# befelix/safe_learning

Hardware: AMD Instinct MI355X
Metric: grid-cell Lyapunov checks/sec + ms/safe_set-update, 4D 128^4 grid, 1k-pt GP (higher is better)
Workload: dtype f64

## Files before the change

### include/sl_hip.h

```cpp
#ifndef SL_HIP_H
#define SL_HIP_H

#include <stdint.h>

#ifdef __cplusplus
extern "C" {
#endif

#define SL_API __attribute__((visibility("default")))

#define SL_OK               0
#define SL_ERR_INVALID     (-1)
#define SL_ERR_HIP         (-2)
#define SL_ERR_UNSUPPORTED (-3)
#define SL_ERR_NOMEM       (-4)

#define SL_MAX_STATE_DIM   6
#define SL_MAX_ACTION_DIM  2
#define SL_MAX_INPUT_DIM   8
#define SL_MAX_GP_HEADS    6
#define SL_MAX_NN_LAYERS   4
#define SL_MAX_SIMPLICES   32

typedef struct sl_ctx sl_ctx;
// ... 107 lines not shown

#define SL_POLYV_MAX_ENTRIES 256
SL_API int  sl_value_polynomial_set(sl_ctx* ctx, int d, int nterms, const double* h_coef,
                    const uint8_t* h_exponents, int normalize, const double* h_tx);

SL_API int  sl_gp_set_head(sl_ctx* ctx, int head, int n, int p, int dout, int col0,
                    const double* h_X, const double* h_Linv, const double* h_alpha,
                    double variance, const double* h_lengthscales);
#define SL_KERNEL_RBF 0
#define SL_KERNEL_MATERN32 1
#define SL_KERNEL_LINEAR 2
#define SL_KERNEL_MAX_FACTORS 8
typedef struct sl_gp_kernel_factor {
    int32_t kind, product;
    double  variance[SL_MAX_INPUT_DIM];
    double  inv_lengthscales[SL_MAX_INPUT_DIM];
} sl_gp_kernel_factor;
typedef struct sl_gp_kernel {
    int32_t nfactors, reserved;
    sl_gp_kernel_factor factor[SL_KERNEL_MAX_FACTORS];
} sl_gp_kernel;
SL_API int  sl_gp_set_head_kernel(sl_ctx* ctx, int head, int n, int p, int dout, int col0,
                    const double* h_X, const double* h_Linv, const double* h_alpha,
                    const sl_gp_kernel* h_kernel);
SL_API int  sl_gp_append_point(sl_ctx* ctx, int head, const double* h_x, const double* h_linv_row,
                        const double* h_alpha_new);
SL_API int  sl_gp_variance_floor(sl_ctx* ctx, int head, double* out, int n);
SL_API int  sl_gp_configure(sl_ctx* ctx, int nheads, double beta);
SL_API int  sl_gp4_early_configure(sl_ctx* ctx, int enable);
SL_API int  sl_gp4_workgroups_configure(sl_ctx* ctx, int workgroups);
SL_API int  sl_gp4_segment_configure(sl_ctx* ctx, int tiles);
SL_API int  sl_gp4_halves_configure(sl_ctx* ctx, int enable);
SL_API int  sl_gp4_predecide_configure(sl_ctx* ctx, int enable, int spacing);

SL_API int  sl_tri_set(sl_ctx* ctx, int slot, const sl_grid_desc* h_grid, int nsimplex,
                const int32_t* h_simplices, const double* h_hyperplanes,
                const double* h_discrete_points, int project, int ncols, const double* d_table);
SL_API int  sl_tri_set_table(sl_ctx* ctx, int slot, const double* d_table);

SL_API int  sl_network_set(sl_ctx* ctx, int nlayers, const int32_t* h_dims ,
                    const int32_t* h_activations, const double* h_kernels);

SL_API int  sl_policy_network_set(sl_ctx* ctx, int nlayers, const int32_t* h_dims,
                           const int32_t* h_activations, const double* h_kernels,
                           const double* h_biases, const int32_t* h_has_bias, double output_scale);

SL_API int  sl_values(sl_ctx* ctx, int64_t lo, int64_t hi, double* d_values);

SL_API int  sl_lyap_sweep(sl_ctx* ctx, int64_t lo, int64_t hi, const uint64_t* d_init_bits,
                   const double* d_values, uint64_t* d_neg_bits, sl_sweep_result* d_result,
                   double* d_dbg);


SL_API int  sl_values_implicit(sl_ctx* ctx, int* out);

SL_API int  sl_fold_results(sl_ctx* ctx, const sl_sweep_result* d_records, int count,
                     sl_sweep_result* d_out);

SL_API int  sl_lyap_finalize_dev(sl_ctx* ctx, int64_t lo, int64_t hi, const double* d_values,
                          const uint64_t* d_init_bits, const uint64_t* d_prev_bits,
                          const sl_sweep_result* d_folded, const sl_key* d_keep,
                          uint64_t* d_safe_bits, sl_sweep_result* d_result);

SL_API int  sl_refinement_carry(sl_ctx* ctx, int64_t lo, int64_t hi, const double* d_values,
                         const uint64_t* d_init_bits, const uint64_t* d_neg_bits,
                         const sl_sweep_result* d_folded, const sl_key* d_keep, int64_t* d_refinement);
// ... 166 lines not shown
```

### safe_learning_amd/_hip.py

```python

import ctypes as C
import os

import numpy as np

HERE = os.path.dirname(os.path.abspath(__file__))
LIB_PATH = os.environ.get("SL_LIB_PATH") or os.path.join(HERE, "libslhip.so")

MAX_STATE_DIM = 6
MAX_ACTION_DIM = 2
MAX_INPUT_DIM = 8
MAX_GP_HEADS = 6
MAX_NN_LAYERS = 4
MAX_SIMPLICES = 32

OK, ERR_INVALID, ERR_HIP, ERR_UNSUPPORTED, ERR_NOMEM = 0, -1, -2, -3, -4
POLICY_LINEAR, POLICY_CONST, POLICY_TABLE, POLICY_TRI, POLICY_NETWORK = 1, 2, 3, 4, 5
DYN_LINEAR, DYN_PENDULUM, DYN_CARTPOLE, DYN_GP, DYN_POLYNOMIAL = 1, 2, 3, 4, 5
POLY_MAX_TERMS, POLY_MAX_DEGREE = 64, 8
V_QUADRATIC, V_TRI, V_NETWORK, V_POLYNOMIAL = 1, 2, 3, 4
POLYV_MAX_ENTRIES = 256
LIP_CONST, LIP_ABS_LINEAR, LIP_NORM_LINEAR, LIP_ABS_GRAD, LIP_NORM_GRAD = 0, 1, 2, 3, 4
LF_CONST, LF_AFFINE_NORM1 = 0, 1
EVAL_VALUE, EVAL_POLICY, EVAL_DYNAMICS, EVAL_DECREASE, EVAL_LV, EVAL_GRADIENT = 1, 2, 3, 4, 5, 6
# ... 87 lines not shown
ADAPTIVE_ROW_WORDS = 6
SELECT_WORDS = 8
S_PREFIX, S_REMAINING, S_KEY_V, S_KEY_I, S_RANK, S_NONE = range(6)

_vp, _i64, _int, _dbl = C.c_void_p, C.c_int64, C.c_int, C.c_double
_int32_p = C.POINTER(C.c_int32)

SIGNATURES = {
    "sl_version": (_int, ()),
    "sl_ctx_create": (_int, (_int, _vp, C.POINTER(_vp))),
    "sl_ctx_destroy": (_int, (_vp,)),
    "sl_last_error": (C.c_char_p, (_vp,)),
    "sl_ctx_synchronize": (_int, (_vp,)),
    "sl_last_kernel": (C.c_char_p, (_vp,)),
    "sl_timing_configure": (_int, (_vp, _int)),
    "sl_timing_collect": (_int, (_vp, _int, c_double_p, _int, C.POINTER(_int))),
    "sl_model_set": (_int, (_vp, C.POINTER(ModelDesc))),
    "sl_policy_touch": (_int, (_vp,)),
    "sl_dynamics_polynomial_set": (_int, (_vp, _int, _int, _int, _int32_p, c_double_p, C.POINTER(C.c_uint8), _int,
                                          _dbl)),
    "sl_value_polynomial_set": (_int, (_vp, _int, _int, c_double_p, C.POINTER(C.c_uint8), _int, c_double_p)),
    "sl_gp_set_head": (_int, (_vp, _int, _int, _int, _int, _int, c_double_p, c_double_p, c_double_p, _dbl,
                              c_double_p)),
    "sl_gp_set_head_kernel": (_int, (_vp, _int, _int, _int, _int, _int, c_double_p, c_double_p, c_double_p,
                                     C.POINTER(GpKernel))),
    "sl_gp_append_point": (_int, (_vp, _int, c_double_p, c_double_p, c_double_p)),
    "sl_gp_variance_floor": (_int, (_vp, _int, c_double_p, _int)),
    "sl_gp_configure": (_int, (_vp, _int, _dbl)),
    "sl_gp4_early_configure": (_int, (_vp, _int)),
    "sl_gp4_workgroups_configure": (_int, (_vp, _int)),
    "sl_gp4_segment_configure": (_int, (_vp, _int)),
    "sl_gp4_halves_configure": (_int, (_vp, _int)),
    "sl_gp4_predecide_configure": (_int, (_vp, _int, _int)),
    "sl_tri_set": (_int, (_vp, _int, C.POINTER(GridDesc), _int, _int32_p, c_double_p, c_double_p, _int, _int,
                          _vp)),
    "sl_tri_set_table": (_int, (_vp, _int, _vp)),
    "sl_network_set": (_int, (_vp, _int, _int32_p, _int32_p, c_double_p)),
    "sl_policy_network_set": (_int, (_vp, _int, _int32_p, _int32_p, c_double_p, c_double_p, _int32_p, _dbl)),
    "sl_values": (_int, (_vp, _i64, _i64, _vp)),
    "sl_lyap_sweep": (_int, (_vp, _i64, _i64, _vp, _vp, _vp, _vp, _vp)),
    "sl_values_implicit": (_int, (_vp, C.POINTER(_int))),
    "sl_fold_results": (_int, (_vp, _vp, _int, _vp)),
    "sl_lyap_finalize_dev": (_int, (_vp, _i64, _i64, _vp, _vp, _vp, _vp, _vp, _vp, _vp)),
    "sl_refinement_carry": (_int, (_vp, _i64, _i64, _vp, _vp, _vp, _vp, _vp, _vp)),
    "sl_select_begin": (_int, (_vp, _vp, _i64, _i64, _vp, _i64)),
    "sl_select_hist": (_int, (_vp, _i64, _i64, _vp, _int, _int, _vp, _vp)),
    "sl_select_digit": (_int, (_vp, _int, _int, _vp, _vp)),
    "sl_sort_pairs": (_int, (_vp, _i64, _vp, _vp, _vp, _vp, _vp)),
    "sl_partition_by_digit": (_int, (_vp, _i64, _vp, _vp, _vp, _vp)),
    "sl_gather_rows": (_int, (_vp, _i64, _int, _vp, _vp, _vp)),
    "sl_adaptive_pack": (_int, (_vp, _i64, _i64, _vp, _vp, _int, _vp, _vp, _vp, _vp)),
    "sl_adaptive_dest": (_int, (_vp, _i64, _vp, _vp, _int, _vp)),
    "sl_adaptive_sort_keys": (_int, (_vp, _i64, _vp, _vp, _vp)),
    "sl_adaptive_analyse": (_int, (_vp, _i64, _i64, _i64, _vp, _vp, _dbl, _dbl, _i64, _vp, _vp)),
    "sl_adaptive_apply": (_int, (_vp, _i64, _i64, _i64, _vp, _vp, _vp, _dbl, _dbl, _i64, _vp)),
    "sl_adaptive_scatter": (_int, (_vp, _i64, _i64, _i64, _vp, _vp, _vp, _vp, _vp)),
    "sl_index_to_state": (_int, (_vp, _i64, _vp, _vp)),
    "sl_perturb_pairs": (_int, (_vp, _i64, _int, _int, _vp, _vp, _int, _vp, _vp, _vp)),
    "sl_rows_sort_key": (_int, (_vp, _i64, _int, _int, _vp, _vp, _vp)),
    "sl_rows_duplicate_flags": (_int, (_vp, _i64, _int, _vp, _vp, _vp)),
    "sl_sample_bounds": (_int, (_vp, _i64, _int, _int, _vp, _vp, _vp, _dbl, _vp, _vp)),
    "sl_state_membership": (_int, (_vp, _i64, _vp, _vp, _vp)),
    "sl_argmax_masked": (_int, (_vp, _i64, _vp, _vp, _vp)),
    "sl_argmax_rows_masked": (_int, (_vp, _i64, _int, _vp, _vp, _i64, _vp)),
    "sl_lyapunov_region": (_int, (_vp, _vp, _i64, _vp, _vp, C.POINTER(_int))),
    "sl_bits_to_bytes": (_int, (_vp, _i64, _vp, _vp)),
# ... 473 lines not shown

    def dense_param_grad(self, dims, activations, has_bias, output_scale, d_params, n, d, d_points, d_coeff, d_out):
        keep, (pd, pa, pb) = self._dense_description(dims, activations, has_bias)
        self.lib.sl_dense_param_grad(self.handle, len(keep[1]), pd, pa, pb, float(output_scale), _ptr(d_params),
                                     int(n), int(d), _ptr(d_points), _ptr(d_coeff), _ptr(d_out))

    def nn_train_scratch(self):
        nbytes, intact = _i64(0), _int(0)
        self.lib.sl_debug_nn_train_scratch(self.handle, C.byref(nbytes), C.byref(intact))
        return int(nbytes.value), bool(intact.value)

    def synchronize(self):
        self.lib.sl_ctx_synchronize(self.handle)

    TIMING_LYAP_SWEEP, TIMING_FINALIZE, TIMING_BELLMAN = 0, 1, 2

    def timing_configure(self, slots):
        self.lib.sl_timing_configure(self.handle, int(slots))
        self._timing_slots = int(slots)

    def timing_collect(self, channel):
        slots = getattr(self, "_timing_slots", 0)
        if not slots:
            return []
        out = (C.c_double * slots)()
        count = C.c_int(0)
        self.lib.sl_timing_collect(self.handle, int(channel), out, slots, C.byref(count))
        return [float(out[i]) for i in range(count.value)]

    def last_kernel(self):
        name = self.lib.sl_last_kernel(self.handle)
        return name.decode() if name else ""

    @staticmethod
    def comm_unique_id():
        lib = load_library()
        buf = C.create_string_buffer(128)
        rc = lib.sl_comm_unique_id(buf)
        if rc != 0:
            raise HipEngineError("sl_comm_unique_id failed: %s" % lib.sl_last_error(None).decode())
        return buf.raw

    def comm_init(self, unique_id, rank, world):
        self.lib.sl_comm_init(self.handle, unique_id, rank, world)

    def comm_destroy(self):
        self.lib.sl_comm_destroy(self.handle)

    def allreduce_result(self, d_result):
        self.lib.sl_allreduce_result(self.handle, _ptr(d_result))

    def allgather(self, d_send, d_recv, nbytes):
        self.lib.sl_allgather(self.handle, _ptr(d_send), _ptr(d_recv), nbytes)

    def allreduce_sum_u64(self, d_values, count):
        self.lib.sl_allreduce_sum_u64(self.handle, _ptr(d_values), count)

    def allreduce_max_f64(self, d_values, count):
        self.lib.sl_allreduce_max_f64(self.handle, _ptr(d_values), count)

    def debug_mfma(self, a, b):
        a, pa = _as_c(a)
        b, pb = _as_c(b)
        out = np.zeros((16, 16))
        self.lib.sl_debug_mfma(self.handle, pa, pb, out.ctypes.data_as(c_double_p))
        return out
# ... 24 lines not shown
```

### safe_learning_amd/csrc/sl_gp4_mean.hip

```cpp
#include "sl_common.h"
#include "sl_gp4_gen.h"
#include "sl_gp4_mean.h"
#include "sl_gp4_predecide.h"
#include "sl_gp4_queue.h"

#ifndef SL_NO_GP4

namespace gp4m {

using gp4::RUNC;
using gp4::RUNS;
using gp4::uniform;

constexpr int W = 4;
constexpr int WG_PER_CU = 4;
constexpr int KXS2 = 128 + 4;
constexpr int KXBUF = 8 * KXS2;
constexpr int SLICE = KXBUF + 16 * SL_P + RUNS * RUNC;
static_assert(16 * SL_D <= KXBUF, "the block's means reuse the chunk buffer");
static_assert(W * SLICE * sizeof(double) <= 40 * 1024, "four workgroups of k_gp_mean_blocks per CU");

}

#ifdef SL_DIAG
static __device__ unsigned long long sl_gp4_mean_decided;
#endif

template <int DT, int MT>
__global__ __launch_bounds__(256, 4) void k_gp_mean_blocks(
    const SlDevModel M, const SlGpDev gp, SlAux aux, int64_t lo, int64_t hi, int64_t tile0, int64_t tile1,
    const uint64_t* __restrict__ init_bits, const double* __restrict__ values,
    uint64_t* __restrict__ neg_bits, sl_key* __restrict__ partials, int fold,
    const double* __restrict__ points, int skip_arg, unsigned long long* __restrict__ ticket,
    unsigned* __restrict__ list_count, long long* __restrict__ list_cell, double* __restrict__ list_mean,
    unsigned list_cap, const unsigned char* __restrict__ pre_tiles) {
#ifdef SL_DIAG
    const int skip = skip_arg;
#else
    constexpr int skip = 0;
    (void)skip_arg;
#endif
    using namespace gp4m;
    __shared__ __attribute__((aligned(16))) double smem[W * SLICE];
    const SlDims nd = sl_dims<DT, MT>(M);
    const int d = nd.d, p = nd.p;
    const int tid = threadIdx.x, lane = tid & 63;
    const int wave = __builtin_amdgcn_readfirstlane(tid >> 6);
    const int lcol = lane & 15, lk = lane >> 4, blk = (lane >> 2) & 3, low = lane & 3;
    double* kx_l = smem + wave * SLICE;
    double* cell_mean = kx_l;
    double* cin = kx_l + KXBUF;
    double* runc = cin + 16 * SL_P;
    const int own = 2 * (16 * lk + ((lcol + 4 * (lk >> 1)) & 15));
// ... 179 lines not shown
                const int64_t b16 = (blk0 - lo) >> 4;
                unsigned init = 0u;
                if (init_bits) init = reinterpret_cast<const unsigned short*>(init_bits)[b16];
                if (lane == 0) reinterpret_cast<unsigned short*>(neg_bits)[b16] = (unsigned short)word;
                const bool okc = neg_hi || ((init >> lcol) & 1u);
                if (valid && !okc) sl_key_min(best_v, best_i, sl_vbits(v_x), idx);
#ifdef SL_DIAG
                if (lane == 0) atomicAdd(&sl_gp4_mean_decided, 1ull);
#endif
            } else {
                unsigned at = 0u;
                if (lane == 0) at = atomicAdd(list_count, 1u);
                at = (unsigned)__builtin_amdgcn_readfirstlane((int)at);
                if (at < list_cap) {
                    if (lane == 0) list_cell[at] = blk0;
                    double* rec = list_mean + (size_t)at * 16 * d;
                    for (int i = lane; i < 16 * d; i += 64) rec[i] = cell_mean[(i / d) * SL_D + i % d];
                }
            }
            __builtin_amdgcn_fence(__ATOMIC_RELEASE, "wavefront");
            __builtin_amdgcn_wave_barrier();
        }
    }
    sl_wave_reduce_key<true>(best_v, best_i);
    if (lane == 0) {
        sl_key* out = partials + blockIdx.x * W + wave;
        if (fold) sl_key_min(best_v, best_i, out->vbits, out->index);
        out->vbits = best_v;
        out->index = best_i;
    }
}

template <int DT, int MT>
static int launch_mean(sl_ctx* ctx, const SlDevModel& model, const SlSweepArgs& a, const Gp4MeanLaunch& m) {
    SlAux aux{ctx->d_tri, ctx->d_net};
    const int skip = sl_diag_flags("SL_GP4_SKIP");
    if (!m.fold) {
        ctx->gp4_pre_tiles = nullptr;
        ctx->gp4_pre_count = nullptr;
        if (sl_gp4_predecide_ok(ctx, model, a)) {
            const Gp4PreLaunch pl{m.workgroups, m.partials, m.ticket + 5};
            const int rc = sl_gp4_predecide_launch_dim<DT>(ctx, model, a, pl, &ctx->gp4_pre_tiles);
            if (rc) return rc;
            ctx->gp4_pre_count = m.ticket + 5;
        }
    }
    const int fold = m.fold || ctx->gp4_pre_tiles != nullptr;
    hipLaunchKernelGGL((k_gp_mean_blocks<DT, MT>), dim3((unsigned)m.workgroups), dim3(gp4m::W * 64), 0, ctx->stream,
                       model, ctx->h_gp, aux, a.lo, a.hi, (int64_t)m.tile0, (int64_t)m.tile1, a.init_bits, a.values,
                       a.neg_bits, m.partials, fold, a.points, skip, m.ticket, m.list_count, m.list_cell,
                       m.list_mean, m.list_cap, ctx->gp4_pre_tiles);
    SL_HIP_CHECK(ctx, hipGetLastError());
    return SL_OK;
}

#if !defined(SL_GP4_DIM) || SL_GP4_DIM == 4
int sl_gp4_mean_workgroups(const sl_ctx* ctx, long long tiles) {
    long long wg = (long long)ctx->num_cu * gp4m::WG_PER_CU;
    const long long need = (tiles + gp4m::W - 1) / gp4m::W;
    if (wg > need) wg = need;
    if (wg > SL_MAX_GRID / 2) wg = SL_MAX_GRID / 2;
    return (int)(wg < 1 ? 1 : wg);
}

unsigned long long sl_gp4_mean_decided_fetch(sl_ctx* ctx) {
    unsigned long long c = 0ull;
#ifdef SL_DIAG
    if (hipMemcpyFromSymbol(&c, HIP_SYMBOL(sl_gp4_mean_decided), sizeof(c)) != hipSuccess) return 0ull;
    const unsigned long long zero = 0ull;
    (void)hipMemcpyToSymbol(HIP_SYMBOL(sl_gp4_mean_decided), &zero, sizeof(zero));
#endif
    (void)ctx;
    return c;
}
#endif

#define SL_GP4_MEAN_ENTRY(D_)                                                                                \
    template <>                                                                                              \
    int sl_gp4_mean_launch_dim<D_>(sl_ctx* ctx, const SlDevModel& model, const SlSweepArgs& a,               \
                                   const Gp4MeanLaunch& m) {                                                 \
// ... 16 lines not shown
```

### safe_learning_amd/csrc/sl_gp4_predecide.h

```cpp
#pragma once
#include "sl_model.h"

namespace gp4p {

constexpr double SLACK = 0x1p-40;
constexpr long long MAX_LATTICE = 1ll << 24;
constexpr long long MAX_TABLE_BYTES = 64ll << 20;

struct PreConst {
    double norm[SL_D], eps[SL_D];
    double sdev;
    int32_t spacing, count[SL_D];
};

SL_HD int row_doubles(int d, int p) { return p + d + d * p; }
SL_HD int lattice_count(int num, int S) { return (num - 1 + S - 1) / S + 1; }
SL_HD int lattice_grid_index(int a, int num, int S) { return a * S < num - 1 ? a * S : num - 1; }
SL_HD int lattice_nearest(int i, int num, int S) {
    const int a = i / S, ia = a * S;
    const int ib = ia + S < num - 1 ? ia + S : num - 1;
    return (i - ia) > (ib - i) ? a + 1 : a;
}

constexpr double HALF_SQRT3 = 0.8660254037844388;
// ... 31 lines not shown
                   0x1p-48 * absm;
            A[j] = fabs(mu[j]) + B[j];
        }
    }
    double vc = 0.0, lin = 0.0, quad = 0.0, mag = 0.0;
#pragma unroll
    for (int j = 0; j < SL_D; ++j) {
        if (j < d) {
            double row = 0.0, grad = 0.0, qb = 0.0, qa = 0.0;
#pragma unroll
            for (int i = 0; i < SL_D; ++i) {
                if (i < d) {
                    row = row + mu[i] * v.matrix[i][j];
                    grad = grad + mu[i] * (v.matrix[i][j] + v.matrix[j][i]);
                    qb = qb + fabs(v.matrix[i][j]) * B[i];
                    qa = qa + fabs(v.matrix[i][j]) * A[i];
                }
            }
            vc = vc + row * mu[j];
            lin = lin + fabs(grad) * B[j];
            quad = quad + qb * B[j];
            mag = mag + qa * A[j];
        }
    }
    mag = mag + fabs(v_x) + fabs(thr);
    const double lower = ((vc - lin) - quad) - v_x;
    return mag < INFINITY && lower >= thr + SLACK * mag;
}

}

#if defined(__HIPCC__)
#include "sl_common.h"

struct Gp4PreLaunch {
    int workgroups;
    sl_key* partials;
    unsigned long long* decided;
};

bool sl_gp4_predecide_ok(const sl_ctx* ctx, const SlDevModel& model, const SlSweepArgs& a);

template <int D>
int sl_gp4_predecide_launch_dim(sl_ctx* ctx, const SlDevModel& model, const SlSweepArgs& a, const Gp4PreLaunch& m,
                                const unsigned char** tiles);
#define SL_GP4_PRE_DECL(D_)                                                                                  \
    template <> int sl_gp4_predecide_launch_dim<D_>(sl_ctx*, const SlDevModel&, const SlSweepArgs&,          \
                                                    const Gp4PreLaunch&, const unsigned char**);
SL_GP4_PRE_DECL(1) SL_GP4_PRE_DECL(2) SL_GP4_PRE_DECL(3) SL_GP4_PRE_DECL(4)
#undef SL_GP4_PRE_DECL
#endif
```

### safe_learning_amd/csrc/sl_gp4_predecide.hip

```cpp
#include "sl_common.h"
#include "sl_gp4_predecide.h"

template <int DT, int MT>
__global__ __launch_bounds__(256) void k_gp_mean_lattice(const SlDevModel M, const SlGpDev gp, SlAux aux,
                                                         const gp4p::PreConst pc, long long npoints,
                                                         double* __restrict__ table) {
    const SlDims nd = sl_dims<DT, MT>(M);
    const int d = nd.d, p = nd.p;
    const SlGpHeadDev& hd = gp.head[0];
    const long long at = (long long)blockIdx.x * blockDim.x + threadIdx.x;
    if (at >= npoints) return;
    long long r = at;
    int64_t cell = 0, stride = 1;
#pragma unroll
    for (int k = SL_D - 1; k >= 0; --k) {
        if (k < d) {
            const int a = (int)(r % pc.count[k]);
            r /= pc.count[k];
            cell += stride * gp4p::lattice_grid_index(a, M.m.grid.num_points[k], pc.spacing);
            stride *= M.m.grid.num_points[k];
        }
    }
    double xg[SL_P], u[SL_M], g[SL_D], J[SL_D][SL_P];
    sl_cell_state(M, d, cell, nullptr, xg);
// ... 81 lines not shown
        double z_c[SL_P], g_c[SL_D], J[SL_D * SL_P];
#pragma unroll
        for (int q = 0; q < SL_P; ++q) z_c[q] = (q < p) ? row[q] : 0.0;
#pragma unroll
        for (int j = 0; j < SL_D; ++j) g_c[j] = (j < d) ? row[p + j] : 0.0;
#pragma unroll
        for (int i = 0; i < SL_D * SL_P; ++i) J[i] = (i < d * p) ? row[p + d + i] : 0.0;
        const bool sure = valid && gp4p::sure_fail(M.m.value, d, p, pc, z, z_c, g_c, J, prior, v_x, thr);
        const uint64_t ok = __ballot(sure || !valid);
        unsigned dec = 0u;
#pragma unroll
        for (int jb = 0; jb < 4; ++jb)
            if (((ok >> (16 * jb)) & 0xffffull) == 0xffffull) dec |= 1u << jb;
        const bool mine = (dec >> (lane >> 4)) & 1u;
        if (mine && (lane & 15) == 0) reinterpret_cast<unsigned short*>(neg_bits)[4 * t + (lane >> 4)] = (unsigned short)0;
        bool init = false;
        if (init_bits && valid) init = (init_bits[t] >> lane) & 1ull;
        if (valid && mine && !init) sl_key_min(best_v, best_i, sl_vbits(values ? values[idx - lo] : v_x), idx);
        if (lane == 0) tiles[t] = (unsigned char)dec;
        const int64_t left = hi - (lo + 64 * t);
        const unsigned live = left >= 64 ? 15u : (1u << (int)((left + 15) >> 4)) - 1u;
        count += (unsigned)__builtin_popcount(dec & live);
    }
    sl_wave_reduce_key<true>(best_v, best_i);
    if (lane == 0) {
        sl_key* out = partials + blockIdx.x * 4 + wave;
        out->vbits = best_v;
        out->index = best_i;
        if (count) atomicAdd(decided, (unsigned long long)count);
    }
}

#if !defined(SL_GP4_DIM) || SL_GP4_DIM == 4
constexpr int64_t PRE_MIN_TILES = 1 << 15;

bool sl_gp4_predecide_ok(const sl_ctx* ctx, const SlDevModel& model, const SlSweepArgs& a) {
    if (ctx->gp4_segment_tiles <= 0 && (a.hi - a.lo + 63) / 64 < PRE_MIN_TILES) return false;
    if (!ctx->gp4_predecide || ctx->gp4_pre_spacing < 1 || a.points || a.dbg || ctx->h_gp.nheads != 1) return false;
    const SlGpHeadHost& hh = ctx->gp_heads[0];
    if (!hh.set || !hh.mb_ok || hh.d_kernel || hh.col0 != 0 || hh.dout != model.m.grid.d) return false;
    if (model.m.value.kind != SL_V_QUADRATIC || model.m.value.negate) return false;
    if (model.m.policy.kind != SL_POLICY_LINEAR && model.m.policy.kind != SL_POLICY_CONST) return false;
    long long npoints = 1;
    for (int k = 0; k < model.m.grid.d; ++k) {
        if (model.m.grid.num_points[k] < 1) return false;
        npoints *= gp4p::lattice_count((int)model.m.grid.num_points[k], ctx->gp4_pre_spacing);
        if (npoints > gp4p::MAX_LATTICE) return false;
    }
    const int d = model.m.grid.d;
    if (npoints * gp4p::row_doubles(d, model.in_dim) * (long long)sizeof(double) > gp4p::MAX_TABLE_BYTES) return false;
    return true;
}

extern "C" int sl_gp4_predecide_configure(sl_ctx* ctx, int enable, int spacing) {
    if (!ctx) return sl_fail(nullptr, SL_ERR_INVALID, "sl_gp4_predecide_configure: NULL context");
    if (spacing < 0 || spacing > 4096)
        return sl_fail(ctx, SL_ERR_INVALID, "sl_gp4_predecide_configure: spacing %d outside [0,4096]", spacing);
    ctx->gp4_predecide = enable != 0;
    if (spacing > 0) ctx->gp4_pre_spacing = spacing;
    return SL_OK;
}
#endif

template <int DT, int MT>
static int launch_predecide(sl_ctx* ctx, const SlDevModel& model, const SlSweepArgs& a, const Gp4PreLaunch& m,
                            const unsigned char** tiles_out) {
    const SlGpHeadHost& hh = ctx->gp_heads[0];
    gp4p::PreConst pc = {};
    long long npoints = 1;
    for (int k = 0; k < DT; ++k) {
        pc.norm[k] = hh.mb_norm[k];
        pc.eps[k] = hh.mb_eps[k];
        pc.count[k] = gp4p::lattice_count((int)model.m.grid.num_points[k], ctx->gp4_pre_spacing);
        npoints *= pc.count[k];
    }
    pc.spacing = ctx->gp4_pre_spacing;
    pc.sdev = sqrt(ctx->h_gp.head[0].variance) * (1.0 + 0x1p-50);
    const int64_t ntiles = (a.hi - a.lo + 63) / 64;
    const size_t table_bytes = ((size_t)npoints * gp4p::row_doubles(DT, DT + MT) * sizeof(double) + 255) & ~(size_t)255;
    SL_HIP_CHECK(ctx, sl_grow(ctx, &ctx->d_gp4_pre, &ctx->gp4_pre_bytes, table_bytes + (size_t)ntiles + 4));
    double* table = reinterpret_cast<double*>(ctx->d_gp4_pre);
    unsigned char* tiles = reinterpret_cast<unsigned char*>(ctx->d_gp4_pre) + table_bytes;
    SlAux aux{ctx->d_tri, ctx->d_net};
    hipLaunchKernelGGL((k_gp_mean_lattice<DT, MT>), dim3((unsigned)((npoints + 255) / 256)), dim3(256), 0, ctx->stream,
                       model, ctx->h_gp, aux, pc, npoints, table);
    SL_HIP_CHECK(ctx, hipGetLastError());
    hipLaunchKernelGGL((k_gp_predecide<DT, MT>), dim3((unsigned)m.workgroups), dim3(256), 0, ctx->stream, model,
                       ctx->h_gp, aux, pc, a.lo, a.hi, a.init_bits, a.values, a.neg_bits, m.partials, table, tiles,
                       m.decided);
    SL_HIP_CHECK(ctx, hipGetLastError());
    *tiles_out = tiles;
    return SL_OK;
}

#define SL_GP4_PRE_ENTRY(D_)                                                                                 \
    template <>                                                                                              \
    int sl_gp4_predecide_launch_dim<D_>(sl_ctx* ctx, const SlDevModel& model, const SlSweepArgs& a,          \
                                        const Gp4PreLaunch& m, const unsigned char** tiles) {                \
        return launch_predecide<D_, 1>(ctx, model, a, m, tiles);                                             \
    }
#if !defined(SL_GP4_DIM) || SL_GP4_DIM == 1
SL_GP4_PRE_ENTRY(1)
#endif
#if !defined(SL_GP4_DIM) || SL_GP4_DIM == 2
SL_GP4_PRE_ENTRY(2)
#endif
#if !defined(SL_GP4_DIM) || SL_GP4_DIM == 3
SL_GP4_PRE_ENTRY(3)
#endif
#if !defined(SL_GP4_DIM) || SL_GP4_DIM == 4
SL_GP4_PRE_ENTRY(4)
#endif
```

Measured before the change: 313.4 million.

## Compact predecided tiles into an open-block list and sweep only open blocks

After the predecide pass, two new kernels count and scatter the indices of still-open 16-cell blocks into a compact list using a chunked prefix sum. A new k_gp_mean_open kernel walks this list through an atomic ticket, so the expensive GP mean evaluation runs only on undecided blocks rather than scanning every tile and skipping decided ones. This adds two small kernel launches, extra device memory and an indirection, and it changes how tiles are assigned to workgroups. A host API to read back the open list is also added for inspection.

Result: faster. 329.2 million (median of 6 runs) (+5.0%).

```diff
diff --git a/include/sl_hip.h b/include/sl_hip.h
--- a/include/sl_hip.h
+++ b/include/sl_hip.h
@@ -163,6 +163,7 @@
 SL_API int  sl_gp4_segment_configure(sl_ctx* ctx, int tiles);
 SL_API int  sl_gp4_halves_configure(sl_ctx* ctx, int enable);
 SL_API int  sl_gp4_predecide_configure(sl_ctx* ctx, int enable, int spacing);
+SL_API int  sl_gp4_open_list(sl_ctx* ctx, uint32_t* out, int64_t cap, unsigned long long* count, int* used);
 
 SL_API int  sl_tri_set(sl_ctx* ctx, int slot, const sl_grid_desc* h_grid, int nsimplex,
                 const int32_t* h_simplices, const double* h_hyperplanes,
diff --git a/safe_learning_amd/_hip.py b/safe_learning_amd/_hip.py
--- a/safe_learning_amd/_hip.py
+++ b/safe_learning_amd/_hip.py
@@ -143,6 +143,7 @@
     "sl_gp4_segment_configure": (_int, (_vp, _int)),
     "sl_gp4_halves_configure": (_int, (_vp, _int)),
     "sl_gp4_predecide_configure": (_int, (_vp, _int, _int)),
+    "sl_gp4_open_list": (_int, (_vp, C.POINTER(C.c_uint32), _i64, C.POINTER(C.c_ulonglong), C.POINTER(_int))),
     "sl_tri_set": (_int, (_vp, _int, C.POINTER(GridDesc), _int, _int32_p, c_double_p, c_double_p, _int, _int,
                           _vp)),
     "sl_tri_set_table": (_int, (_vp, _int, _vp)),
@@ -682,6 +683,18 @@
         name = self.lib.sl_last_kernel(self.handle)
         return name.decode() if name else ""
 
+    def gp4_open_list(self, entries=True):
+        import numpy as np
+        count, used = C.c_ulonglong(0), C.c_int(0)
+        self.lib.sl_gp4_open_list(self.handle, None, 0, C.byref(count), C.byref(used))
+        if not entries:
+            return int(count.value), bool(used.value)
+        out = np.zeros(int(count.value), dtype=np.uint32)
+        if len(out):
+            self.lib.sl_gp4_open_list(self.handle, out.ctypes.data_as(C.POINTER(C.c_uint32)), len(out),
+                                      C.byref(count), C.byref(used))
+        return out, bool(used.value)
+
     @staticmethod
     def comm_unique_id():
         lib = load_library()
diff --git a/safe_learning_amd/csrc/sl_gp4_mean.hip b/safe_learning_amd/csrc/sl_gp4_mean.hip
--- a/safe_learning_amd/csrc/sl_gp4_mean.hip
+++ b/safe_learning_amd/csrc/sl_gp4_mean.hip
@@ -19,6 +19,9 @@
 constexpr int SLICE = KXBUF + 16 * SL_P + RUNS * RUNC;
 static_assert(16 * SL_D <= KXBUF, "the block's means reuse the chunk buffer");
 static_assert(W * SLICE * sizeof(double) <= 40 * 1024, "four workgroups of k_gp_mean_blocks per CU");
+constexpr int KEYS = 2 * 16;
+constexpr int SLICE_OPEN = SLICE + KEYS;
+static_assert(W * SLICE_OPEN * sizeof(double) <= 40 * 1024, "four workgroups of k_gp_mean_open per CU");
 
 }
 
@@ -264,6 +267,251 @@
 }
 
 template <int DT, int MT>
+__global__ __launch_bounds__(256, 4) void k_gp_mean_open(
+    const SlDevModel M, const SlGpDev gp, SlAux aux, int64_t lo, int64_t hi, unsigned p0, unsigned p1,
+    const unsigned* __restrict__ open_list, const unsigned long long* __restrict__ open_len,
+    const uint64_t* __restrict__ init_bits, const double* __restrict__ values,
+    uint64_t* __restrict__ neg_bits, sl_key* __restrict__ partials,
+    const double* __restrict__ points, int skip_arg, unsigned* __restrict__ ticket,
+    unsigned* __restrict__ list_count, long long* __restrict__ list_cell, double* __restrict__ list_mean,
+    unsigned list_cap) {
+#ifdef SL_DIAG
+    const int skip = skip_arg;
+#else
+    constexpr int skip = 0;
+    (void)skip_arg;
+#endif
+    using namespace gp4m;
+    __shared__ __attribute__((aligned(16))) double smem[W * SLICE_OPEN];
+    const SlDims nd = sl_dims<DT, MT>(M);
+    const int d = nd.d, p = nd.p;
+    const int tid = threadIdx.x, lane0 = tid & 63;
+    const int wave = __builtin_amdgcn_readfirstlane(tid >> 6);
+    double* kx_l = smem + wave * SLICE_OPEN;
+    double* cell_mean = kx_l;
+    double* cin = kx_l + KXBUF;
+    double* runc = cin + 16 * SL_P;
+    uint64_t* keys = reinterpret_cast<uint64_t*>(runc + RUNS * RUNC);
+    if (lane0 < 16) {
+        keys[2 * lane0] = ~0ull;
+        keys[2 * lane0 + 1] = (uint64_t)INT64_MAX;
+    }
+
+    const SlGpHeadDev& hd = gp.head[0];
+    const int n_pad = hd.n_pad, dout = hd.dout;
+    const double variance = hd.variance;
+    __amdgpu_buffer_rsrc_t rs_xs = __builtin_amdgcn_make_buffer_rsrc((void*)hd.xs, 0, 0x7fffffff, 0x27000);
+    __amdgpu_buffer_rsrc_t rs_alpha = __builtin_amdgcn_make_buffer_rsrc((void*)hd.alpha, 0, 0x7fffffff, 0x27000);
+    constexpr int RP = 256;
+    const int npanels = (hd.n + RP - 1) / RP;
+    const int nchunks_head = npanels * (RP / 64);
+
+    {
+        const unsigned long long len = open_len[0];
+        if (len < (unsigned long long)p1) p1 = (unsigned)len;
+    }
+    if (p0 >= p1) return;
+    auto request = [&]() -> unsigned {
+        unsigned t = 0u;
+        if (lane0 == 0) t = atomicInc(ticket, 0xffffffffu);
+        return t;
+    };
+    unsigned drawn = request();
+    for (;;) {
+        asm volatile("" : "+v"(drawn));
+        const unsigned pos = p0 + 4u * (unsigned)__builtin_amdgcn_readfirstlane((int)drawn);
+        if (pos >= p1) break;
+        drawn = request();
+        const sl_u4 entry = *reinterpret_cast<const sl_u4*>(open_list + pos);
+        const int nb = p1 - pos < 4u ? (int)(p1 - pos) : 4;
+        for (int jb = 0; jb < nb; ++jb) {
+            const unsigned b16 = jb == 0 ? entry.x : jb == 1 ? entry.y : jb == 2 ? entry.z : entry.w;
+            const int64_t blk0 = lo + 16 * (int64_t)b16;
+            int lane = lane0;
+            asm volatile("" : "+v"(lane));
+            const int lcol = lane & 15, lk = lane >> 4, blk = (lane >> 2) & 3, low = lane & 3;
+            const int own = 2 * (16 * lk + ((lcol + 4 * (lk >> 1)) & 15));
+            const int wbase = (lane >> 3) * KXS2 + 32 * (lane & 3) + ((lane >> 2) & 1);
+            const int wswz = 4 * ((lane & 3) >> 1);
+            if (lk == 0) {
+                double xg[SL_P], u[SL_M];
+                int64_t gidx = blk0 + lcol;
+                gidx = gidx < hi ? gidx : hi - 1;
+                sl_cell_state(M, d, gidx, points, xg);
+                sl_policy_any<false>(M, nd, aux.tri, gidx, xg, u);
+                sl_append_action(nd, u, xg);
+#pragma unroll
+                for (int q = 0; q < SL_P; ++q) cin[lcol * SL_P + q] = (q < p) ? xg[q] * hd.inv_ls[q] : 0.0;
+            }
+            __builtin_amdgcn_fence(__ATOMIC_RELEASE, "wavefront");
+            __builtin_amdgcn_wave_barrier();
+            unsigned runs = 1u;
+            bool wide = false;
+            {
+                bool bend = false;
+                if (lcol >= 1) {
+                    double st2 = 0.0;
+#pragma unroll
+                    for (int q = 0; q < SL_P; ++q) {
+                        if (q < p) {
+                            const double st = cin[lcol * SL_P + q] - cin[(lcol - 1) * SL_P + q];
+                            st2 = fma(st, st, st2);
+                        }
+                    }
+                    wide = !(st2 <= 1.0);
+                }
+                if (lcol >= 2) {
+#pragma unroll
+                    for (int q = 0; q < SL_P; ++q) {
+                        if (q < p) {
+                            const double c0 = cin[lcol * SL_P + q];
+                            const double c1 = cin[(lcol - 1) * SL_P + q];
+                            const double c2 = cin[(lcol - 2) * SL_P + q];
+                            bend = bend || fabs((c0 - c1) - (c1 - c2)) > 2e-14 * fmax(1.0, fabs(c0));
+                        }
+                    }
+                }
+                unsigned bends = (unsigned)(__ballot(bend) & 0xffffull);
+                while (bends) {
+                    const int c = __builtin_ctz(bends);
+                    runs |= 1u << c;
+                    bends &= ~(3u << c);
+                }
+            }
+            runs = (unsigned)__builtin_amdgcn_readfirstlane((int)runs);
+            const bool direct = __builtin_popcount(runs) > 4 || (__ballot(wide) & 0xffffull) != 0ull;
+            if (!direct || runs == 1u) {
+                if (lane < RUNS) {
+                    unsigned m = runs;
+                    for (int r = 0; r < lane; ++r) m &= m - 1;
+                    if (m) {
+                        const int c0 = __builtin_ctz(m);
+                        m &= m - 1;
+                        const int c1 = m ? __builtin_ctz(m) : 16;
+                        const double* at = cin + c0 * SL_P;
+                        const bool single = c1 - c0 < 2;
+                        double a2r = 0.0;
+                        double* rc = runc + lane * RUNC;
+#pragma unroll
+                        for (int q = 0; q < SL_P; ++q) {
+                            const double step = (q < p && !single) ? at[SL_P + q] - at[q] : 0.0;
+                            rc[q] = step;
+                            a2r = fma(step, step, a2r);
+                        }
+                        rc[SL_P] = a2r;
+                        rc[SL_P + 1] = sl_exp_nonpos(-a2r);
+                    }
+                }
+                __builtin_amdgcn_fence(__ATOMIC_RELEASE, "wavefront");
+                __builtin_amdgcn_wave_barrier();
+            }
+            double macc[4] = {0.0, 0.0, 0.0, 0.0};
+
+            auto generate = [&](int ch) {
+                double* kxw = kx_l + wbase;
+                double xv[SL_P];
+#pragma unroll
+                for (int q = 0; q < SL_P; ++q)
+                    if (q < p)
+                        xv[q] = __builtin_bit_cast(double, __builtin_amdgcn_raw_buffer_load_b64(
+                            rs_xs, lane * 8, (q * n_pad + 64 * ch) * 8, 0));
+                if (runs == 1u) {
+                    double e, rho;
+                    gp4::run_seed(xv, cin, runc, variance, p, e, rho);
+                    gp4::store_run16(kxw, wswz, rho, e, runc[SL_P + 1]);
+                } else if (!direct) {
+                    unsigned m = runs;
+                    for (int r = 0; m; ++r) {
+                        const int c0 = __builtin_ctz(m);
+                        m &= m - 1;
+                        const int c1 = m ? __builtin_ctz(m) : 16;
+                        const double* rc = runc + r * RUNC;
+                        double e, rho;
+                        gp4::run_seed(xv, cin + c0 * SL_P, rc, variance, p, e, rho);
+                        const double qr = rc[SL_P + 1];
+                        for (int c = c0; c < c1; ++c) {
+                            kxw[2 * ((c + wswz) & 15)] = e;
+                            e *= rho;
+                            rho *= qr;
+                        }
+                    }
+                } else {
+                    gp4::direct_run(kxw, wswz, xv, cin, 0, variance, p);
+                }
+            };
+            for (int ch = 0; ch < nchunks_head; ++ch) {
+                const bool with_mean = !(skip & 2);
+                gp4::MeanIn mi;
+                if (with_mean) gp4::load_alpha(mi, rs_alpha, lk, low, dout, ch);
+                if (!(skip & 1)) generate(ch);
+                if (with_mean) {
+                    __builtin_amdgcn_fence(__ATOMIC_RELEASE, "wavefront");
+                    __builtin_amdgcn_wave_barrier();
+                    sl_d2 kx[8];
+                    gp4::load_own_kx<KXS2>(kx, kx_l + own);
+                    gp4::mean_mfma(kx, mi, macc);
+                }
+            }
+            __builtin_amdgcn_fence(__ATOMIC_RELEASE, "wavefront");
+            __builtin_amdgcn_wave_barrier();
+            if (lk < dout) cell_mean[(4 * blk + low) * SL_D + hd.col0 + lk] = gp4::mean_sum(macc);
+            __builtin_amdgcn_fence(__ATOMIC_RELEASE, "wavefront");
+            __builtin_amdgcn_wave_barrier();
+
+            const int64_t idx = blk0 + lcol;
+            const bool valid = lk == 0 && idx < hi;
+            gp4::CellBounds b{false, false, 0.0};
+            if (valid)
+                b = gp4::cell_bounds<false>(M, nd, aux, gp.beta, idx, lo, points, values, cell_mean + lcol * SL_D, variance,
+                                            0.0, 0.0);
+            const bool neg_hi = b.neg_hi, open = b.open;
+            const double v_x = b.v_x;
+            if (__ballot(open) == 0ull) {
+                const unsigned word = (unsigned)(__ballot(neg_hi) & 0xffffull);
+                unsigned init = 0u;
+                if (init_bits) init = reinterpret_cast<const unsigned short*>(init_bits)[b16];
+                if (lane == 0) reinterpret_cast<unsigned short*>(neg_bits)[b16] = (unsigned short)word;
+                const bool okc = neg_hi || ((init >> lcol) & 1u);
+                if (valid && !okc) {
+                    uint64_t best_v = keys[2 * lcol];
+                    int64_t best_i = (int64_t)keys[2 * lcol + 1];
+                    sl_key_min(best_v, best_i, sl_vbits(v_x), idx);
+                    keys[2 * lcol] = best_v;
+                    keys[2 * lcol + 1] = (uint64_t)best_i;
+                }
+#ifdef SL_DIAG
+                if (lane == 0) atomicAdd(&sl_gp4_mean_decided, 1ull);
+#endif
+            } else {
+                unsigned at = 0u;
+                if (lane == 0) at = atomicAdd(list_count, 1u);
+                at = (unsigned)__builtin_amdgcn_readfirstlane((int)at);
+                if (at < list_cap) {
+                    if (lane == 0) list_cell[at] = blk0;
+                    double* rec = list_mean + (size_t)at * 16 * d;
+                    for (int i = lane; i < 16 * d; i += 64) rec[i] = cell_mean[(i / d) * SL_D + i % d];
+                }
+            }
+            __builtin_amdgcn_fence(__ATOMIC_RELEASE, "wavefront");
+            __builtin_amdgcn_wave_barrier();
+        }
+    }
+    uint64_t best_v = ~0ull;
+    int64_t best_i = INT64_MAX;
+    if (lane0 < 16) {
+        best_v = keys[2 * lane0];
+        best_i = (int64_t)keys[2 * lane0 + 1];
+    }
+    sl_wave_reduce_key<true>(best_v, best_i);
+    if (lane0 == 0) {
+        sl_key* out = partials + blockIdx.x * W + wave;
+        sl_key_min(best_v, best_i, out->vbits, out->index);
+        out->vbits = best_v;
+        out->index = best_i;
+    }
+}
+
+template <int DT, int MT>
 static int launch_mean(sl_ctx* ctx, const SlDevModel& model, const SlSweepArgs& a, const Gp4MeanLaunch& m) {
     SlAux aux{ctx->d_tri, ctx->d_net};
     const int skip = sl_diag_flags("SL_GP4_SKIP");
@@ -278,6 +526,17 @@
         }
     }
     const int fold = m.fold || ctx->gp4_pre_tiles != nullptr;
+    const long long ntiles = (long long)((a.hi - a.lo + 63) / 64);
+    if (ctx->gp4_pre_tiles && sl_gp4_open_fits(ntiles)) {
+        const Gp4OpenView ov = sl_gp4_open_view(ctx->gp4_pre_tiles, ntiles);
+        hipLaunchKernelGGL((k_gp_mean_open<DT, MT>), dim3((unsigned)m.workgroups), dim3(gp4m::W * 64), 0, ctx->stream,
+                           model, ctx->h_gp, aux, a.lo, a.hi, (unsigned)(4 * m.tile0), (unsigned)(4 * m.tile1),
+                           (const unsigned*)ov.list, (const unsigned long long*)(ov.head + gp4o::HEAD_LENGTH),
+                           a.init_bits, a.values, a.neg_bits, m.partials, a.points, skip,
+                           reinterpret_cast<unsigned*>(m.ticket), m.list_count, m.list_cell, m.list_mean, m.list_cap);
+        SL_HIP_CHECK(ctx, hipGetLastError());
+        return SL_OK;
+    }
     hipLaunchKernelGGL((k_gp_mean_blocks<DT, MT>), dim3((unsigned)m.workgroups), dim3(gp4m::W * 64), 0, ctx->stream,
                        model, ctx->h_gp, aux, a.lo, a.hi, (int64_t)m.tile0, (int64_t)m.tile1, a.init_bits, a.values,
                        a.neg_bits, m.partials, fold, a.points, skip, m.ticket, m.list_count, m.list_cell,
diff --git a/safe_learning_amd/csrc/sl_gp4_open.h b/safe_learning_amd/csrc/sl_gp4_open.h
--- /dev/null
+++ b/safe_learning_amd/csrc/sl_gp4_open.h
@@ -0,0 +1,53 @@
+#pragma once
+#include <stddef.h>
+#include <stdint.h>
+
+#ifndef SL_HD
+#if defined(__HIPCC__) || defined(__CUDACC__)
+#define SL_HD __host__ __device__ __forceinline__
+#else
+#define SL_HD inline
+#endif
+#endif
+
+namespace gp4o {
+
+constexpr int CHUNK_TILES = 4096;
+constexpr int HEAD_BYTES = 64;
+constexpr int HEAD_LENGTH = 0, HEAD_NTILES = 1, HEAD_BUILT = 2;
+
+SL_HD int popcount32(uint32_t v) {
+#if defined(__HIP_DEVICE_COMPILE__)
+    return __popc(v);
+#else
+    return __builtin_popcount(v);
+#endif
+}
+
+SL_HD uint32_t open_nibble(uint32_t byte) { return ~byte & 15u; }
+
+SL_HD uint32_t open_mask16(uint32_t word, int valid) {
+    uint32_t m = 0u;
+    for (int k = 0; k < 4; ++k)
+        if (k < valid) m |= open_nibble((word >> (8 * k)) & 255u) << (4 * k);
+    return m;
+}
+
+SL_HD uint32_t open_count(const unsigned char* bytes, long long n) {
+    uint32_t c = 0u;
+    for (long long t = 0; t < n; ++t) c += (uint32_t)popcount32(open_nibble(bytes[t]));
+    return c;
+}
+
+SL_HD uint32_t open_rank(const unsigned char* bytes, long long t, int jb) {
+    return open_count(bytes, t) + (uint32_t)popcount32(open_nibble(bytes[t]) & ((1u << jb) - 1u));
+}
+
+SL_HD long long chunks(long long ntiles) { return (ntiles + CHUNK_TILES - 1) / CHUNK_TILES; }
+SL_HD size_t tile_bytes(long long ntiles) { return ((size_t)ntiles + 4 + 15) & ~(size_t)15; }
+SL_HD size_t count_bytes(long long ntiles) { return ((size_t)chunks(ntiles) * 4 + 15) & ~(size_t)15; }
+SL_HD size_t total_bytes(long long ntiles) {
+    return HEAD_BYTES + tile_bytes(ntiles) + count_bytes(ntiles) + 16 * (size_t)ntiles;
+}
+
+}
diff --git a/safe_learning_amd/csrc/sl_gp4_predecide.h b/safe_learning_amd/csrc/sl_gp4_predecide.h
--- a/safe_learning_amd/csrc/sl_gp4_predecide.h
+++ b/safe_learning_amd/csrc/sl_gp4_predecide.h
@@ -87,6 +87,23 @@
 
 #if defined(__HIPCC__)
 #include "sl_common.h"
+#include "sl_gp4_open.h"
+
+struct Gp4OpenView {
+    unsigned long long* head;
+    unsigned* counts;
+    unsigned* list;
+};
+inline Gp4OpenView sl_gp4_open_view(const unsigned char* tiles, long long ntiles) {
+    unsigned char* t = const_cast<unsigned char*>(tiles);
+    Gp4OpenView v;
+    v.head = reinterpret_cast<unsigned long long*>(t - gp4o::HEAD_BYTES);
+    v.counts = reinterpret_cast<unsigned*>(t + gp4o::tile_bytes(ntiles));
+    v.list = reinterpret_cast<unsigned*>(t + gp4o::tile_bytes(ntiles) + gp4o::count_bytes(ntiles));
+    return v;
+}
+inline bool sl_gp4_open_fits(long long ntiles) { return 4 * ntiles < (1ll << 31); }
+int sl_gp4_open_build(sl_ctx* ctx, const unsigned char* tiles, long long ntiles);
 
 struct Gp4PreLaunch {
     int workgroups;
diff --git a/safe_learning_amd/csrc/sl_gp4_predecide.hip b/safe_learning_amd/csrc/sl_gp4_predecide.hip
--- a/safe_learning_amd/csrc/sl_gp4_predecide.hip
+++ b/safe_learning_amd/csrc/sl_gp4_predecide.hip
@@ -137,6 +137,81 @@
 }
 
 #if !defined(SL_GP4_DIM) || SL_GP4_DIM == 4
+namespace gp4o {
+constexpr int LANES = 256;
+constexpr int ROUNDS = CHUNK_TILES / (4 * LANES);
+static_assert(ROUNDS * 4 * LANES == CHUNK_TILES, "a chunk is a whole number of rounds");
+
+__device__ __forceinline__ uint32_t lane_mask(const unsigned* __restrict__ words, long long ntiles, long long chunk,
+                                              int r, long long& t) {
+    t = chunk * CHUNK_TILES + 4 * (long long)(r * LANES + (int)threadIdx.x);
+    if (t >= ntiles) return 0u;
+    const long long left = ntiles - t;
+    return open_mask16(words[t >> 2], left < 4 ? (int)left : 4);
+}
+__device__ __forceinline__ unsigned group_sum(unsigned v, unsigned* part) {
+#pragma unroll
+    for (int off = 32; off >= 1; off >>= 1) v += __shfl_xor(v, off);
+    __syncthreads();
+    if ((threadIdx.x & 63) == 0) part[threadIdx.x >> 6] = v;
+    __syncthreads();
+    return part[0] + part[1] + part[2] + part[3];
+}
+}
+
+__global__ __launch_bounds__(256) void k_gp_open_count(const unsigned* __restrict__ words, long long ntiles,
+                                                       unsigned* __restrict__ counts) {
+    __shared__ unsigned part[4];
+    unsigned c = 0u;
+#pragma unroll
+    for (int r = 0; r < gp4o::ROUNDS; ++r) {
+        long long t;
+        c += (unsigned)__popc(gp4o::lane_mask(words, ntiles, blockIdx.x, r, t));
+    }
+    c = gp4o::group_sum(c, part);
+    if (threadIdx.x == 0) counts[blockIdx.x] = c;
+}
+
+__global__ __launch_bounds__(256) void k_gp_open_scatter(const unsigned* __restrict__ words, long long ntiles,
+                                                         const unsigned* __restrict__ counts,
+                                                         unsigned* __restrict__ list,
+                                                         unsigned long long* __restrict__ head) {
+    __shared__ unsigned part[4];
+    const int lane = threadIdx.x & 63, wave = threadIdx.x >> 6;
+    unsigned before = 0u;
+    for (unsigned i = threadIdx.x; i < blockIdx.x; i += gp4o::LANES) before += counts[i];
+    unsigned base = gp4o::group_sum(before, part);
+    for (int r = 0; r < gp4o::ROUNDS; ++r) {
+        long long t;
+        uint32_t m = gp4o::lane_mask(words, ntiles, blockIdx.x, r, t);
+        const unsigned n = (unsigned)__popc(m);
+        unsigned incl = n;
+#pragma unroll
+        for (int off = 1; off < 64; off <<= 1) {
+            const unsigned up = __shfl_up(incl, off);
+            if (lane >= off) incl += up;
+        }
+        __syncthreads();
+        if (lane == 63) part[wave] = incl;
+        __syncthreads();
+        unsigned at = base + incl - n;
+        for (int w = 0; w < wave; ++w) at += part[w];
+        while (m) {
+            const int i = __builtin_ctz(m);
+            m &= m - 1u;
+            list[at++] = (unsigned)(4 * t) + (unsigned)i;
+        }
+        base += part[0] + part[1] + part[2] + part[3];
+    }
+    if (blockIdx.x == gridDim.x - 1 && threadIdx.x == 0) {
+        head[gp4o::HEAD_LENGTH] = base;
+        head[gp4o::HEAD_NTILES] = (unsigned long long)ntiles;
+        head[gp4o::HEAD_BUILT] = 1ull;
+    }
+}
+#endif
+
+#if !defined(SL_GP4_DIM) || SL_GP4_DIM == 4
 constexpr int64_t PRE_MIN_TILES = 1 << 15;
 
 bool sl_gp4_predecide_ok(const sl_ctx* ctx, const SlDevModel& model, const SlSweepArgs& a) {
@@ -165,6 +240,37 @@
     if (spacing > 0) ctx->gp4_pre_spacing = spacing;
     return SL_OK;
 }
+int sl_gp4_open_build(sl_ctx* ctx, const unsigned char* tiles, long long ntiles) {
+    const Gp4OpenView v = sl_gp4_open_view(tiles, ntiles);
+    const unsigned nchunks = (unsigned)gp4o::chunks(ntiles);
+    const unsigned* words = reinterpret_cast<const unsigned*>(tiles);
+    hipLaunchKernelGGL(k_gp_open_count, dim3(nchunks), dim3(gp4o::LANES), 0, ctx->stream, words, ntiles, v.counts);
+    SL_HIP_CHECK(ctx, hipGetLastError());
+    hipLaunchKernelGGL(k_gp_open_scatter, dim3(nchunks), dim3(gp4o::LANES), 0, ctx->stream, words, ntiles, v.counts,
+                       v.list, v.head);
+    SL_HIP_CHECK(ctx, hipGetLastError());
+    return SL_OK;
+}
+
+extern "C" int sl_gp4_open_list(sl_ctx* ctx, uint32_t* out, int64_t cap, unsigned long long* count, int* used) {
+    if (!ctx) return sl_fail(nullptr, SL_ERR_INVALID, "sl_gp4_open_list: NULL context");
+    if (cap < 0 || (cap && !out)) return sl_fail(ctx, SL_ERR_INVALID, "sl_gp4_open_list: bad output (cap %lld)", (long long)cap);
+    if (count) *count = 0ull;
+    if (used) *used = 0;
+    if (!ctx->gp4_pre_tiles || !strstr(ctx->last_kernel, "after k_gp_mean_blocks")) return SL_OK;
+    SL_HIP_CHECK(ctx, hipSetDevice(ctx->device));
+    SL_HIP_CHECK(ctx, hipStreamSynchronize(ctx->stream));
+    unsigned long long head[3] = {0ull, 0ull, 0ull};
+    SL_HIP_CHECK(ctx, hipMemcpy(head, ctx->gp4_pre_tiles - gp4o::HEAD_BYTES, sizeof(head), hipMemcpyDeviceToHost));
+    if (head[gp4o::HEAD_BUILT] != 1ull) return SL_OK;
+    const Gp4OpenView v = sl_gp4_open_view(ctx->gp4_pre_tiles, (long long)head[gp4o::HEAD_NTILES]);
+    const unsigned long long n = head[gp4o::HEAD_LENGTH];
+    if (count) *count = n;
+    if (used) *used = 1;
+    const size_t take = n < (unsigned long long)cap ? (size_t)n : (size_t)cap;
+    if (take) SL_HIP_CHECK(ctx, hipMemcpy(out, v.list, take * sizeof(uint32_t), hipMemcpyDeviceToHost));
+    return SL_OK;
+}
 #endif
 
 template <int DT, int MT>
@@ -183,9 +289,10 @@
     pc.sdev = sqrt(ctx->h_gp.head[0].variance) * (1.0 + 0x1p-50);
     const int64_t ntiles = (a.hi - a.lo + 63) / 64;
     const size_t table_bytes = ((size_t)npoints * gp4p::row_doubles(DT, DT + MT) * sizeof(double) + 255) & ~(size_t)255;
-    SL_HIP_CHECK(ctx, sl_grow(ctx, &ctx->d_gp4_pre, &ctx->gp4_pre_bytes, table_bytes + (size_t)ntiles + 4));
+    SL_HIP_CHECK(ctx, sl_grow(ctx, &ctx->d_gp4_pre, &ctx->gp4_pre_bytes, table_bytes + gp4o::total_bytes(ntiles)));
     double* table = reinterpret_cast<double*>(ctx->d_gp4_pre);
-    unsigned char* tiles = reinterpret_cast<unsigned char*>(ctx->d_gp4_pre) + table_bytes;
+    unsigned char* tiles = reinterpret_cast<unsigned char*>(ctx->d_gp4_pre) + table_bytes + gp4o::HEAD_BYTES;
+    SL_HIP_CHECK(ctx, hipMemsetAsync(tiles - gp4o::HEAD_BYTES, 0, gp4o::HEAD_BYTES, ctx->stream));
     SlAux aux{ctx->d_tri, ctx->d_net};
     hipLaunchKernelGGL((k_gp_mean_lattice<DT, MT>), dim3((unsigned)((npoints + 255) / 256)), dim3(256), 0, ctx->stream,
                        model, ctx->h_gp, aux, pc, npoints, table);
@@ -195,6 +302,7 @@
                        m.decided);
     SL_HIP_CHECK(ctx, hipGetLastError());
     *tiles_out = tiles;
+    if (sl_gp4_open_fits(ntiles)) return sl_gp4_open_build(ctx, tiles, ntiles);
     return SL_OK;
 }
 
```
